# ChanghyeonKim93/bundle_adjustment_solver

Hardware: AMD Instinct MI355X
Metric: lm_iterations_per_sec (higher is better)
Workload: dtype f64; 1 GPU; C4 stereo 6-DoF: 1000 poses / 500k landmarks / 5M obs; n_opt_poses=995, n_opt_landmarks=500000, n_observations=5000000, parallelism=single GPU, exchange=none

## Files before the change

bundle_adjustment_solver_amd/_lib.py:

```python
import ctypes as C
import os

_HERE = os.path.dirname(os.path.abspath(__file__))
LIB_PATH = os.environ.get("BA_HIP_LIB") or os.path.join(_HERE, "libba_hip.so")


class BaOptions(C.Structure):
    _fields_ = [
        ("threshold_step_size", C.c_float),
        ("threshold_cost_change", C.c_float),
        ("threshold_huber_loss", C.c_float),
        ("threshold_outlier_rejection", C.c_float),
        ("max_num_iterations", C.c_int),
        ("initial_lambda", C.c_float),
        ("decrease_ratio_lambda", C.c_float),
        ("increase_ratio_lambda", C.c_float),
        ("gauss_newton", C.c_int),
    ]


def make_options(max_iter=50, thr_step=1e-5, thr_cost=1e-5, huber=1.0,
                 outlier=2.0, lambda0=100.0, dec=0.33, inc=3.0,
                 gauss_newton=False):
    o = BaOptions()
# ... 99 lines not shown
    "ba_solve_gd": (C.c_int, [_P, C.POINTER(BaOptions), C.POINTER(BaIterInfo),
                              C.c_int, C.POINTER(C.c_int), C.POINTER(C.c_int)]),
    "ba_gd_get_gradient": (C.c_int, [_P, _D, _D]),
    "ba_stage_cost": (C.c_int, [_P, _D]),
    "ba_stage_linearize": (C.c_int, [_P, C.c_double, C.c_double]),
    "ba_stage_schur": (C.c_int, [_P]),
    "ba_stage_solve_reduced": (C.c_int, [_P]),
    "ba_stage_backsub_update": (C.c_int, [_P]),
    "ba_stage_scalars": (C.c_int, [_P, _D, _D, _D, _D]),
    "ba_stage_commit": (C.c_int, [_P, C.c_int]),
    "ba_enable_stage_timing": (C.c_int, [_P, C.c_int]),
    "ba_get_stage_ms": (C.c_int, [_P, _D, C.c_int]),
    "ba_num_opt_poses": (C.c_int, [_P]),
    "ba_num_opt_points": (C.c_int, [_P]),
    "ba_num_pairs": (C.c_int64, [_P]),
    "ba_num_schur_blocks": (C.c_int64, [_P]),
    "ba_num_schur_triples": (C.c_int64, [_P]),
    "ba_get_poses": (C.c_int, [_P, _D]),
    "ba_get_points": (C.c_int, [_P, _D, _U8]),
    "ba_get_A": (C.c_int, [_P, _D, _D]),
    "ba_get_C": (C.c_int, [_P, _D, _D]),
    "ba_get_Cinv": (C.c_int, [_P, _D, _D]),
    "ba_get_pairs": (C.c_int, [_P, _I32, _I32, _D]),
    "ba_get_S": (C.c_int, [_P, _D, _D]),
    "ba_get_xy": (C.c_int, [_P, _D, _D]),
    "ba_kernel_count": (C.c_int, []),
    "ba_kernel_name": (C.c_char_p, [C.c_int]),
    "ba_get_kernel_ms": (C.c_int, [_P, _D, C.POINTER(C.c_int64), C.c_int]),
    "ba_get_dense_info": (C.c_int, [_P, _D]),
    "ba_get_schur_info": (C.c_int, [_P, C.POINTER(C.c_int64)]),
    "ba_get_lin_info": (C.c_int, [_P, C.POINTER(C.c_int64)]),
    "ba_get_mask_info": (C.c_int, [_P, C.POINTER(C.c_int64)]),
    "ba_get_dropped_pivots": (C.c_int, [_P, C.POINTER(C.c_int64), C.c_int]),
    "ba_dense_spd_solve": (C.c_int, [_P, C.c_int, _D, _D, _D, _D]),
    "ba_pose_only_mono6": (C.c_int, [_P, _F, _F, C.c_int, C.c_float, C.c_float,
                                     C.c_float, C.c_float, _F, _U8,
                                     C.POINTER(BaOptions), C.POINTER(BaPoIter),
                                     C.c_int, C.POINTER(C.c_int),
                                     C.POINTER(C.c_int), _F]),
    "ba_pose_only_stereo6": (C.c_int, [_P, _F, _F, _F, C.c_int, _F, _F, _F, _F,
                                       _U8, _U8, C.POINTER(BaOptions),
                                       C.POINTER(BaPoIter), C.c_int,
                                       C.POINTER(C.c_int), C.POINTER(C.c_int),
                                       _F]),
    "ba_pose_only_mono3": (C.c_int, [_P, _F, _F, C.c_int, C.c_float, C.c_float,
                                     C.c_float, C.c_float, _F, _F, _F, _U8,
                                     C.POINTER(BaOptions), C.POINTER(BaPoIter),
                                     C.c_int, C.POINTER(C.c_int),
                                     C.POINTER(C.c_int), _F]),
    "ba_pose_only_stereo3": (C.c_int, [_P, _F, _F, _F, C.c_int, _F, _F, _F, _F,
                                       _F, _F, _U8, _U8, C.POINTER(BaOptions),
                                       C.POINTER(BaPoIter), C.c_int,
                                       C.POINTER(C.c_int), C.POINTER(C.c_int),
                                       _F]),
    "ba_pose_only_mono6_batch": (C.c_int, [_P, C.c_int, _I32, _F, _F, _F, _F, _U8,
                                           C.POINTER(BaOptions), C.POINTER(BaPoIter),
                                           C.c_int, C.POINTER(BaPoResult), _F]),
    "ba_pose_only_stereo6_batch": (C.c_int, [_P, C.c_int, _I32, _F, _F, _F, _F, _F,
                                             _F, _F, _U8, _U8, C.POINTER(BaOptions),
                                             C.POINTER(BaPoIter), C.c_int,
                                             C.POINTER(BaPoResult), _F]),
    "ba_pose_only_mono6_batch_device": (C.c_int, [_P, C.c_int, _P, _P, _P, _P, _P, _P,
                                                  C.POINTER(BaOptions), _P, C.c_int,
                                                  _P, _P, _P]),
    "ba_pose_only_stereo6_batch_device": (C.c_int, [_P, C.c_int, _P, _P, _P, _P, _P, _P,
                                                    _P, _P, _P, C.POINTER(BaOptions),
# ... 69 lines not shown
```

bundle_adjustment_solver_amd/csrc/ba_api.hip:

```cpp
#include <hip/hip_runtime.h>

#include <algorithm>
#include <chrono>
#include <cmath>
#include <cstdio>
#include <cstdlib>
#include <cstring>
#include <string>
#include <vector>

#include "ba_handle.h"

namespace {
thread_local std::string g_err;
}
void ba::set_last_error(const std::string &m) { g_err = m; }
int ba::fail(const std::string &m) {
  g_err = m;
  return -1;
}
using ba::fail;

namespace {

// ... 493 lines not shown
    if (h->dalloc(&d.grp_pat, pl.grp_pat.size() / 2) || h->upload(&d.pose_gpart_ptr, pl.pose_gpart_ptr) ||
        h->upload(&d.pose_gpart, pl.pose_gpart))
      return -1;
    h->kind(2);
    if (h->dalloc(&d.Apart2, (size_t)pl.n_apart2 * 27) || h->dalloc(&d.lin_dump, (size_t)ba::kLinDump)) return -1;
    if (!pl.grp_pat.empty())
      HIP_TRY(hipMemcpy(d.grp_pat, pl.grp_pat.data(), pl.grp_pat.size() * sizeof(int32_t), hipMemcpyHostToDevice));
    if (pl.n_apart2 > 0) HIP_TRY(hipMemset(d.Apart2, 0, (size_t)pl.n_apart2 * 27 * sizeof(double)));
  }

  lap("structure uploads");
  for (int k = 0; k < 2; ++k) {
    h->kind(2);
    if (h->dalloc(&d.Cu[k], (size_t)pl.M * 6) || h->dalloc(&d.b[k], (size_t)pl.M * 3) ||
        h->dalloc(&d.W[k], std::max<size_t>(2, (size_t)pl.P * ba::kWStride)))
      return -1;
    h->kind(0);
    if (h->dalloc(&d.A[k], (size_t)pl.N * 36) || h->dalloc(&d.a[k], (size_t)pl.N * 6)) return -1;
    HIP_TRY(hipMemset(d.W[k], 0, std::max<size_t>(1, (size_t)pl.P * ba::kWStride) * sizeof(double)));
    HIP_TRY(hipMemset(d.A[k], 0, std::max<size_t>(1, (size_t)pl.N * 36) * sizeof(double)));
    HIP_TRY(hipMemset(d.a[k], 0, std::max<size_t>(1, (size_t)pl.N * 6) * sizeof(double)));
  }
  d.n_obs_lm = pl.M > 0 ? pl.lm_obs_ptr[pl.M] : 0;
  h->kind(2);
  if (h->dalloc(&d.Cd, (size_t)pl.M * 6) || h->dalloc(&d.Cinv, (size_t)pl.M * 6) ||
      h->dalloc(&d.lin_cost_part, (size_t)std::max(1, d.n_lin_cost)) ||
      h->dalloc(&d.Apart, (size_t)d.n_achunk * 27) ||
      h->dalloc(&d.spart, (size_t)d.n_tchunk * ba::kSlotStride) ||
      h->dalloc(&d.y, (size_t)pl.M * 3) || h->dalloc(&d.lm_part, (size_t)std::max(1, d.n_lm_part) * 2))
    return -1;
  h->kind(0);
  if (h->dalloc(&d.x, (size_t)pl.N * 6 + 64) || h->dalloc(&d.cost_part, (size_t)ba::kCostGrid) ||
      h->dalloc(&d.pose_part, (size_t)2 + 2 * ba::kPoseGrid) ||
      h->dalloc(&d.scal, (size_t)4) || h->dalloc(&d.ctrl, (size_t)1))
    return -1;
  HIP_TRY(hipMemset(d.lin_cost_part, 0, (size_t)std::max(1, d.n_lin_cost) * sizeof(double)));
  HIP_TRY(hipMemset(d.x, 0, ((size_t)pl.N * 6 + 64) * sizeof(double)));
  HIP_TRY(hipMemset(d.y, 0, std::max<size_t>(1, (size_t)pl.M * 3) * sizeof(double)));
  HIP_TRY(hipMemset(d.cost_part, 0, ba::kCostGrid * sizeof(double)));
  HIP_TRY(hipMemset(d.lm_part, 0, (size_t)std::max(1, d.n_lm_part) * 2 * sizeof(double)));
  HIP_TRY(hipMemset(d.pose_part, 0, (2 + 2 * ba::kPoseGrid) * sizeof(double)));
  HIP_TRY(hipMemset(d.scal, 0, 4 * sizeof(double)));
  d.log_cap = 4096;
  if (h->dalloc(&d.log, (size_t)d.log_cap)) return -1;

  lap("block storage");
  if (h->dense_owner) {
    const ba_handle *o = h->dense_owner;
    if (!o->finalized || o->plan.N != pl.N || o->plan.B != pl.B)
      return fail("ba_finalize: the dense owner belongs to a different problem");
    h->sched = o->sched;
    h->ddev = o->ddev;
    h->pose_col_h = o->pose_col_h;
    d.nb = o->d.nb; d.npad = o->d.npad; d.ld = o->d.ld;
    d.L = o->d.L; d.Ldiag = o->d.Ldiag; d.pose_col = o->d.pose_col; d.col_x = o->d.col_x;
    d.zt_I = o->d.zt_I; d.zt_J = o->d.zt_J; d.n_zt = o->d.n_zt;
    d.x = o->d.x;
    h->xbuf_n[0] = pl.B * 36 + 6 * (int64_t)pl.N;
    h->xbuf_n[1] = 4;
    h->xbuf_n[2] = 3 * (int64_t)pl.n_pt_global;
    if (h->dalloc(&d.Spk, (size_t)h->xbuf_n[0])) return -1;
    HIP_TRY(hipMemset(d.Spk, 0, (size_t)h->xbuf_n[0] * sizeof(double)));
  } else {
    const char *nat = getenv("BA_DENSE_NATURAL");
    const char *full = getenv("BA_DENSE_FULL");
    const char *force = getenv("BA_DENSE_NB");
    ba::DenseSchedule cand[2];
    double cost[2];
// ... 805 lines not shown
  for (const auto &g : pl.lin_desc) obs += (int64_t)g.nl * g.no;
  out4[0] = (int64_t)pl.lin_desc.size();
  out4[1] = obs;
  out4[2] = (int64_t)pl.bchunk_lm.size() - 1 - (pl.lin_groups ? pl.n_bchunk_grp : 0);
  out4[3] = pl.n_pobs;
  return 0;
}

int ba_get_mask_info(ba_handle *h, int64_t out4[4]) {
  if (!h || !h->finalized || !out4) return fail("ba_get_mask_info: bad argument");
  const ba::Plan &pl = h->plan;
  int64_t lm = 0;
  for (const auto &g : pl.grp_range) lm += g.masked ? g.nl : 0;
  out4[0] = (int64_t)pl.lin_desc.size() - pl.n_lin_plain;
  out4[1] = lm;
  out4[2] = pl.n_obs - (pl.n_obs_global > 0 && h->world == 1 ? pl.n_obs_global : pl.n_obs);
  {
    int64_t pad = 0;
    for (int64_t s2 = 0; s2 < pl.n_obs; ++s2) pad += !(pl.obs_uv[2 * s2] == pl.obs_uv[2 * s2]);
    out4[2] = pad;
  }
  out4[3] = pl.n_pair_pad;
  return 0;
}

int ba_get_dropped_pivots(ba_handle *h, int64_t *count, int reset) {
  if (!h || !h->finalized || !count) return fail("ba_get_dropped_pivots: bad argument");
  if (use_device(h)) return -1;
  int v = 0;
  HIP_TRY(hipMemcpyAsync(&v, h->ddev.bad_pivots, sizeof(int), hipMemcpyDeviceToHost, h->stream));
  if (reset) HIP_TRY(hipMemsetAsync(h->ddev.bad_pivots, 0, sizeof(int), h->stream));
  HIP_TRY(hipStreamSynchronize(h->stream));
  *count = v % ba::kFlowTimeout;
  return 0;
}

int ba_dense_spd_solve(ba_handle *h, int n, const double *A, const double *b,
                       double *x, double *ms) {
  if (!h || n <= 0 || !A || !b || !x) return fail("ba_dense_spd_solve: bad argument");
  if (use_device(h)) return -1;
  const int nb = 64;
  const int ncb = (n + nb - 1) / nb;
  const int npad = ncb * nb;
  const int ld = npad + nb;
  std::vector<uint8_t> adj((size_t)ncb * ncb, 0);
  for (int I = 0; I < ncb; ++I)
    for (int J = 0; J < I; ++J) {
      bool any = false;
      for (int r = I * nb; r < std::min(n, (I + 1) * nb) && !any; ++r)
        for (int c = J * nb; c < (J + 1) * nb && !any; ++c) any = A[(size_t)r * n + c] != 0.0;
      adj[(size_t)I * ncb + J] = adj[(size_t)J * ncb + I] = any;
    }
  ba::DenseSchedule sc;
  const char *nat = getenv("BA_DENSE_NATURAL");
  ba::build_dense_schedule(ncb, adj, nat && atoi(nat) != 0, nb, sc);
  std::vector<int> colmap(npad), col_x(npad, -1);
  for (int c = 0; c < npad; ++c) colmap[c] = sc.pos_of_tile[c / nb] * nb + c % nb;
  std::vector<double> L((size_t)npad * ld, 0.0);
  for (int c = 0; c < npad; ++c) {
    if (c < n) {
      col_x[colmap[c]] = c;
      for (int r = c; r < n; ++r) {
        int rr = colmap[r], cc = colmap[c];
        if (rr < cc) std::swap(rr, cc);
        L[(size_t)cc * ld + rr] = A[(size_t)r * n + c];
      }
// ... 532 lines not shown
```

bundle_adjustment_solver_amd/csrc/ba_device.h:

```cpp
#ifndef BA_DEVICE_H_
#define BA_DEVICE_H_

#include <hip/hip_runtime.h>
#include <stdint.h>
#include <stdlib.h>

#include <vector>

namespace ba {

struct DevCtrl {
  double lambda;
  double prev_cost;
  double huber;
  double thr_step;
  double thr_cost;
  double dec_ratio;
  double inc_ratio;
  unsigned long long t_last;
  int cur;
  int done;
  int iter;
  int converged;
  int max_iter;
// ... 57 lines not shown
    int32_t pat0;
    int32_t apart0, cost_idx;
    int32_t pad_;
  };
  LinDesc *lin_desc;
  int n_lin_desc;
  int n_lin_plain;
  GrpDesc *grp32, *grp64, *grp128;
  int n_grp32, n_grp64, n_grp128;
  int2 *grp_pat;
  double *Apart2;
  double *lin_dump;
  int32_t *pose_gpart_ptr, *pose_gpart;
  int lin_chunk0;
  int n_lin_cost;
  int n_bs_grp;
  int n_lm_part;
  SupDesc *sup_desc;
  uint32_t *sup_lane;
  ChunkDesc *chunk_desc;
  uint16_t *chunk_sp;
  uint32_t *ltri;
  int64_t *blk_contrib_ptr;
  int32_t *contrib_slot;
  int32_t *blk_desc;
  double *spart2;
  double *Cu[2];
  double *b[2];
  double *W[2];
  double *A[2];
  double *a[2];
  double *Cinv;
  double *Cd;
  double *Apart;
  double *spart;
  double *x;
  double *y;
  double *cost_part;
  double *lin_cost_part;
  int64_t n_obs_lm;
  double *lm_part;
  double *pose_part;
  double *scal;
  DevCtrl *ctrl;
  DevIterRec *log;
  int log_cap;
  double *Spk;
  double *L;
  int npad, ld;
  double *Ldiag;
  int nb;
  int *pose_col;
  int *col_x;
  int32_t *bchunk_lm;
  struct LmChunk {
    int64_t pb, ob;
    int32_t l0, nl, np, no;
  };
  LmChunk *lm_chunk;
  int n_bchunk;
  int *zt_I, *zt_J;
  int n_zt;
};

constexpr int kLinDump = 64 * 4 * 4;
constexpr int kFlowTimeout = 1 << 20;
// ... 175 lines not shown
```

bundle_adjustment_solver_amd/csrc/ba_kernels.hip:

```cpp
#include "ba_device.h"
#include "ba_plan.h"

namespace ba {

thread_local KernelTimer *g_ktimer = nullptr;

void KernelTimer::begin(int id, hipStream_t s) {
  const size_t k = ids.size();
  while (pool.size() < 2 * (k + 1)) {
    hipEvent_t e;
    if (hipEventCreate(&e) != hipSuccess) return;
    pool.push_back(e);
  }
  ids.push_back(id);
  (void)hipEventRecord(pool[2 * k], s);
}
void KernelTimer::end(hipStream_t s) {
  if (ids.empty()) return;
  (void)hipEventRecord(pool[2 * (ids.size() - 1) + 1], s);
}
void KernelTimer::collect() {
  for (size_t k = 0; k < ids.size(); ++k) {
    float t = 0.f;
    if (hipEventElapsedTime(&t, pool[2 * k], pool[2 * k + 1]) == hipSuccess) {
// ... 245 lines not shown
  }
  o[0] = b00; o[1] = b01; o[2] = b02; o[3] = b11; o[4] = b12; o[5] = b22;
}

__device__ __forceinline__ double rcp_newton(double d) {
  double r = __builtin_amdgcn_rcp(d);
  r = fma(fma(-d, r, 1.0), r, r);
  r = fma(fma(-d, r, 1.0), r, r);
  return r;
}
__device__ __forceinline__ void spd3_inverse(const double c[6], double o[6]) {
  const double a00 = c[0], a01 = c[1], a02 = c[2], a11 = c[3], a12 = c[4], a22 = c[5];
  const double thr = 1e-6 * fmax(a00, fmax(a11, a22));
  const double i0 = rcp_newton(a00);
  const double l10 = a01 * i0, l20 = a02 * i0;
  const double d1 = fma(-l10, a01, a11);
  const double t21 = fma(-l20, a01, a12);
  const double i1 = rcp_newton(d1);
  const double l21 = t21 * i1;
  const double d2 = fma(-l21, t21, fma(-l20, a02, a22));
  const double i2 = rcp_newton(d2);
  if (!(a00 > thr && d1 > thr && d2 > thr) || !(thr > 0.0)) {
    ldlt3_inverse(c, o);
    return;
  }
  const double m20 = fma(l10, l21, -l20);
  const double w2 = m20 * i2, v2 = l21 * i2;
  o[5] = i2;
  o[4] = -v2;
  o[2] = w2;
  o[3] = fma(l21, v2, i1);
  o[1] = fma(-l10, i1, -(l21 * w2));
  o[0] = fma(m20, w2, fma(l10 * l10, i1, i0));
}

template <bool SLIM>
struct ObsRec;
template <>
struct ObsRec<true> {
  int2 v;
  __device__ __forceinline__ int cam() const { return v.x & 0xffff; }
  __device__ __forceinline__ int pose() const { return (int)((unsigned)v.x >> 16); }
  __device__ __forceinline__ int pt() const { return v.y; }
  __device__ __forceinline__ void load(const DevProblem &d, int64_t s) { v = d.obs_cp[s]; }
  __device__ __forceinline__ void clear() { v = make_int2(0, 0); }
};
template <>
struct ObsRec<false> {
  int4 v;
  __device__ __forceinline__ int cam() const { return v.x; }
  __device__ __forceinline__ int pose() const { return v.y; }
  __device__ __forceinline__ int pt() const { return v.z; }
  __device__ __forceinline__ void load(const DevProblem &d, int64_t s) { v = d.obs_idx[s]; }
  __device__ __forceinline__ void clear() { v = make_int4(0, 0, 0, 0); }
};

#define COST_STEP(TC, XC, TN, XN)                                               \
  {                                                                             \
             \
    const double *Tp_ = poses + (size_t)idn.pose() * 12;                        \
    const double *Xp_ = pts + (size_t)idn.pt() * 3;                             \
    _Pragma("unroll") for (int k_ = 0; k_ < 12; ++k_) TN[k_] = Tp_[k_];         \
    _Pragma("unroll") for (int k_ = 0; k_ < 3; ++k_) XN[k_] = Xp_[k_];          \
    const int ncam_ = idn.cam();                                                \
    const double2 nuv_ = uvn;                                                   \
     \
// ... 870 lines not shown
    }
    if (k < 18) acc[k] = a2; else racc[k - 18] = a2;
  }
#ifdef BA_SCHUR_DBG
  if (dbg_on)
    for (int k = 0; k < 160; ++k) g_schur_dbg[dbg_slot][k] = k < dbg_n ? dbg_s[k] : 0;
#endif
  if (owner && sub2 == 0) {
    double *o = d.spart2 + (size_t)(sd.s0 + slot) * kSlotStride;
#pragma unroll
    for (int k = 0; k < 18; ++k) o[h * 18 + k] = acc[k];
#pragma unroll
    for (int k = 0; k < 3; ++k) o[36 + h * 3 + k] = racc[k];
  }
}

#ifndef BA_GRP_KRW
#define BA_GRP_KRW 36
#endif
#ifdef BA_GRP_DBG
__device__ long long g_grp_dbg[256];
#define GRP_STAMP() { if (gdbg_on && gdbg_n < 256) gdbg_s[gdbg_n++] = clock64(); }
#else
#define GRP_STAMP()
#endif
template <int NT>
__global__ __launch_bounds__(kBlock, (NT == 2 && BA_GRP_KRW <= 24) ? 3 : 2) void k_schur_grp(DevProblem d, const DevProblem::GrpDesc *grps) {
  constexpr int TW = 16 * NT;
#ifndef BA_GRP_KRW
#define BA_GRP_KRW 36
#endif
  constexpr int KRW = NT == 2 ? BA_GRP_KRW : 20;
  constexpr int NTILE = NT * (NT + 1) / 2;
  constexpr int RS = 2 * TW + (NT == 2 ? 6 : 0);
  constexpr int IMG = (KRW / 2) * RS;
  __shared__ __attribute__((aligned(16))) double VA[4][IMG];
  __shared__ __attribute__((aligned(16))) double WB[4][IMG];
  static_assert(IMG >= 256, "the final reduction uses VA as 4 x 256 doubles");
#ifdef BA_GRP_DBG
  __shared__ long long gdbg_s[256];
  const bool gdbg_on = blockIdx.x == 600 && threadIdx.x == 0;
  int gdbg_n = 0;
#endif
  const int tid = threadIdx.x, lane = tid & 63, wv = tid >> 6;
  const int lr = lane & 15, lk = lane >> 4;
  const DevProblem::GrpDesc gd = grps[blockIdx.x];
  const int done = d.ctrl->done;
  const int lb = d.ctrl->lcur;
  BA_KEEP_S(gd.l0);
  BA_KEEP_S(done);
  if (done) return;
  const double *__restrict__ Wg = d.W[lb];
  const double *__restrict__ bg = d.b[lb];
  const double *__restrict__ Cug = d.Cu[lb];
  const double lp1 = 1.0 + d.ctrl->lambda;
  const int dd = gd.d;
  const int nlw = min(64 / dd, KRW / 3);
  const int il = lane / dd, jj = lane - il * dd;
  const int nch = (gd.nl + nlw - 1) / nlw;
  double *va = VA[wv], *wb = WB[wv];
  for (int e = lane; e < IMG; e += 64) {
    va[e] = 0.0;
    wb[e] = 0.0;
  }
  double2 rw[2][6], rc[2][3];
  double rb[2][3];
#define GRP_PREFETCH(B, ch_)                                                        \
  {                                                                                 \
    const int c0_ = (ch_) * nlw;                                                    \
    const bool on_ = il < min(nlw, gd.nl - c0_);                                    \
    const double2 *wp_ = (const double2 *)(Wg + (size_t)(gd.p0 + (int64_t)c0_ * dd + (on_ ? lane : 0)) * kWStride); \
    const int lm_ = gd.l0 + c0_ + (on_ ? il : 0);                                   \
    const double2 *cp_ = (const double2 *)(Cug + (size_t)lm_ * 6);                  \
    _Pragma("unroll") for (int k_ = 0; k_ < 6; ++k_) rw[B][k_] = wp_[k_];           \
    _Pragma("unroll") for (int k_ = 0; k_ < 3; ++k_) rc[B][k_] = cp_[k_];           \
    _Pragma("unroll") for (int k_ = 0; k_ < 3; ++k_) rb[B][k_] = bg[(size_t)lm_ * 3 + k_]; \
  }
  v4f64 acc[NTILE];
#pragma unroll
  for (int t = 0; t < NTILE; ++t) acc[t] = (v4f64){0.0, 0.0, 0.0, 0.0};
  if (wv < nch) GRP_PREFETCH(0, wv)
  if (wv + 4 < nch) GRP_PREFETCH(1, wv + 4)
#define GRP_IDX(k_, col_) (((k_) >> 1) * RS + (col_) * 2 + ((k_) & 1))
#define GRP_STAGE(B)                                                                \
  if (ch < nch) {                                                                   \
    GRP_STAMP()                                                                     \
    const int nlc = min(nlw, gd.nl - ch * nlw);                                     \
    if (il < nlc) {                                                                 \
       \
      _Pragma("clang fp contract(fast)")                                            \
      const double k9[9] = {rw[B][0].x, rw[B][0].y, rw[B][1].x, rw[B][1].y, rw[B][2].x, \
                            rw[B][2].y, rw[B][3].x, rw[B][3].y, rw[B][4].x};        \
      const double x0 = rw[B][4].y, x1 = rw[B][5].x, x2 = rw[B][5].y;               \
          \
      const double cd_[6] = {rc[B][0].x * lp1, rc[B][0].y, rc[B][1].x, rc[B][1].y * lp1, rc[B][2].x, rc[B][2].y * lp1}; \
      double c6[6];                                                                 \
      spd3_inverse(cd_, c6);                                                        \
      double w[18];                                                                 \
      _Pragma("unroll") for (int e = 0; e < 9; ++e) w[e] = k9[e];                   \
      _Pragma("unroll") for (int c = 0; c < 3; ++c) {                               \
        w[9 + c] = x1 * k9[6 + c] - x2 * k9[3 + c];                                 \
        w[12 + c] = x2 * k9[c] - x0 * k9[6 + c];                                    \
        w[15 + c] = x0 * k9[3 + c] - x1 * k9[c];                                    \
      }                                                                             \
      const int kb = 3 * il, cb = 6 * jj;                                           \
      const int i0 = GRP_IDX(kb, cb), i1 = GRP_IDX(kb + 1, cb), i2 = GRP_IDX(kb + 2, cb); \
      _Pragma("unroll") for (int r = 0; r < 6; ++r) {                               \
        const double w0 = w[r * 3], w1 = w[r * 3 + 1], w2 = w[r * 3 + 2];           \
        va[i0 + 2 * r] = w0 * c6[0] + w1 * c6[1] + w2 * c6[2];                      \
        va[i1 + 2 * r] = w0 * c6[1] + w1 * c6[3] + w2 * c6[4];                      \
        va[i2 + 2 * r] = w0 * c6[2] + w1 * c6[4] + w2 * c6[5];                      \
        wb[i0 + 2 * r] = w0;                                                        \
        wb[i1 + 2 * r] = w1;                                                        \
        wb[i2 + 2 * r] = w2;                                                        \
      }                                                                             \
      if (jj == 0) {                           \
        wb[GRP_IDX(kb, 6 * dd)] = rb[B][0];                                         \
        wb[GRP_IDX(kb + 1, 6 * dd)] = rb[B][1];                                     \
        wb[GRP_IDX(kb + 2, 6 * dd)] = rb[B][2];                                     \
      }                                                                             \
    }                                                                               \
    const int nks = (3 * nlc + 3) >> 2;                                             \
    if (nlc < nlw) {  \
      for (int e = lane; e < (4 * nks - 3 * nlc) * TW; e += 64) {                   \
        const int k_ = 3 * nlc + e / TW, c_ = e - (e / TW) * TW;                    \
        va[GRP_IDX(k_, c_)] = 0.0;                                                  \
        wb[GRP_IDX(k_, c_)] = 0.0;                                                  \
      }                                                                             \
    }                                                                               \
    GRP_STAMP()                                                                     \
    if (ch + 8 < nch) GRP_PREFETCH(B, ch + 8)                                       \
    GRP_STAMP()                                                                     \
    __builtin_amdgcn_fence(__ATOMIC_RELEASE, "wavefront");                          \
    __builtin_amdgcn_wave_barrier();                                                \
    __builtin_amdgcn_fence(__ATOMIC_ACQUIRE, "wavefront");                          \
    {                                                                               \
       \
      const double *ap = va + (lk >> 1) * RS + lr * 2 + (lk & 1);                   \
      const double *bp = wb + (lk >> 1) * RS + lr * 2 + (lk & 1);                   \
      double a[NT], b[NT], an[NT], bn[NT];                                          \
      _Pragma("unroll") for (int t = 0; t < NT; ++t) {                              \
        a[t] = ap[32 * t];                                                          \
        b[t] = bp[32 * t];                                                          \
      }                                                                             \
      for (int ks = 0; ks < nks; ++ks) {                                            \
        const int kn = ks + 1 < nks ? ks + 1 : ks;  \
        _Pragma("unroll") for (int t = 0; t < NT; ++t) {                            \
          an[t] = ap[kn * 2 * RS + 32 * t];                                         \
          bn[t] = bp[kn * 2 * RS + 32 * t];                                         \
        }                                                                           \
        int tile = 0;                                                               \
        _Pragma("unroll") for (int ti = 0; ti < NT; ++ti)                           \
        _Pragma("unroll") for (int tj = ti; tj < NT; ++tj) {                        \
          acc[tile] = __builtin_amdgcn_mfma_f64_16x16x4f64(a[ti], b[tj], acc[tile], 0, 0, 0); \
          ++tile;                                                                   \
        }                                                                           \
        _Pragma("unroll") for (int t = 0; t < NT; ++t) {                            \
          a[t] = an[t];                                                             \
          b[t] = bn[t];                                                             \
        }                                                                           \
      }                                                                             \
    }                                                                               \
    __builtin_amdgcn_fence(__ATOMIC_RELEASE, "wavefront");                          \
    __builtin_amdgcn_wave_barrier();                                                \
    __builtin_amdgcn_fence(__ATOMIC_ACQUIRE, "wavefront");                          \
    GRP_STAMP()                                                                     \
    ch += 4;                                                                        \
  }
  for (int ch = wv; ch < nch;) {
    GRP_STAGE(0)
    GRP_STAGE(1)
  }
#undef GRP_STAGE
#undef GRP_IDX
#undef GRP_PREFETCH
  GRP_STAMP()
#ifdef BA_GRP_DBG
  if (gdbg_on) for (int q = 0; q < 256; ++q) g_grp_dbg[q] = q < gdbg_n ? gdbg_s[q] : 0;
#endif
  __syncthreads();
  double *R = &VA[0][0];
  int tile = 0;
#pragma unroll
  for (int ti = 0; ti < NT; ++ti)
#pragma unroll
    for (int tj = ti; tj < NT; ++tj) {
#pragma unroll
      for (int g = 0; g < 4; ++g) R[wv * 256 + g * 64 + lane] = acc[tile][g];
      __syncthreads();
      {
        const double v = ((R[tid] + R[256 + tid]) + R[512 + tid]) + R[768 + tid];
        const int g = tid >> 6, ln = tid & 63;
        const int row = 16 * ti + (ln >> 4) + 4 * g;
        const int col = 16 * tj + (ln & 15);
        const int pj = row / 6, r = row - 6 * pj;
        if (pj < dd) {
          const int sj = gd.s0 + pj * dd - (pj * (pj - 1)) / 2;
          if (col == 6 * dd) {
            d.spart2[(size_t)sj * kSlotStride + 36 + r] = v;
          } else if (col < 6 * dd) {
            const int pk = col / 6, c = col - 6 * pk;
            if (pk >= pj) d.spart2[(size_t)(sj + (pk - pj)) * kSlotStride + r * 6 + c] = v;
          }
        }
      }
      __syncthreads();
      ++tile;
    }
}

#define GW_LDS_BARRIER() asm volatile("s_waitcnt lgkmcnt(0)\n\ts_barrier" ::: "memory")
__global__ __launch_bounds__(kBlock, 2) void k_schur_grp_wide(DevProblem d, const DevProblem::GrpDesc *grps) {
  constexpr int TW = 128;
  constexpr int LPW = 2;
// ... 1441 lines not shown
```

bundle_adjustment_solver_amd/solver.py:

```python
import ctypes as C
import enum
import sys
import time

import numpy as np

from . import _lib
from ._lib import BaIterInfo, BaOptions, BaPoIter, BaPoResult, check

SCALER = 0.01
INVERSE_SCALER = 1.0 / SCALER


class SolverType(enum.IntEnum):
    UNDEFINED = -1
    GRADIENT_DESCENT = 0
    GAUSS_NEWTON = 1
    LEVENBERG_MARQUARDT = 2


class IterationStatus(enum.IntEnum):
    UNDEFINED = -1
    UPDATE = 0
    UPDATE_TRUST_MORE = 1
# ... 426 lines not shown
        return {self.lib.ba_kernel_name(k).decode(): (float(ms[k]), int(calls[k]))
                for k in range(n)}

    def get_dense_info(self):
        out = np.zeros(4)
        check(self.lib.ba_get_dense_info(self.h, _dp(out)),
              "ba_get_dense_info")
        return dict(fill=out[0], flops=out[1], levels=int(out[2]),
                    npad=int(out[3]))

    def get_schur_info(self):
        v = (C.c_int64 * 8)()
        check(self.lib.ba_get_schur_info(self.h, v), "ba_get_schur_info")
        return dict(groups32=int(v[0]), groups64=int(v[1]), grouped_landmarks=int(v[2]),
                    super_runs=int(v[3]), grouped_pairs=int(v[4]), grouped_triples=int(v[5]),
                    group_mfma=int(v[6]), list_triples=int(v[7]))

    def get_lin_info(self):
        v = (C.c_int64 * 4)()
        check(self.lib.ba_get_lin_info(self.h, v), "ba_get_lin_info")
        return dict(group_pieces=int(v[0]), group_observations=int(v[1]), chunks=int(v[2]),
                    pose_major_observations=int(v[3]))

    def get_mask_info(self):
        v = (C.c_int64 * 4)()
        check(self.lib.ba_get_mask_info(self.h, v), "ba_get_mask_info")
        return dict(masked_pieces=int(v[0]), masked_landmarks=int(v[1]),
                    padded_observation_slots=int(v[2]), padded_pairs=int(v[3]))

    def get_dropped_pivots(self, reset=False):
        v = C.c_int64(0)
        check(self.lib.ba_get_dropped_pivots(self.h, C.byref(v), int(reset)),
              "ba_get_dropped_pivots")
        return int(v.value)

    def dense_spd_solve(self, A, b):
        A = np.ascontiguousarray(A, np.float64)
        b = np.ascontiguousarray(b, np.float64)
        n = A.shape[0]
        x = np.zeros(n)
        ms = C.c_double(0)
        check(self.lib.ba_dense_spd_solve(self.h, n, _dp(A), _dp(b), _dp(x),
                                          C.byref(ms)), "ba_dense_spd_solve")
        return x, ms.value

    def pose_only_mono6(self, X3, uv2, fx, fy, cx, cy, T12, mask, opt,
                        cap=None, want_debug=False):
        X = np.ascontiguousarray(X3, np.float32).reshape(-1, 3)
        uv = np.ascontiguousarray(uv2, np.float32).reshape(-1, 2)
        n = X.shape[0]
        T = np.ascontiguousarray(T12, np.float32).reshape(12).copy()
        m = np.ascontiguousarray(mask, np.uint8).copy()
        cap = cap or max(1, opt.max_num_iterations)
        rows = (BaPoIter * cap)()
        n_it = C.c_int(0)
        conv = C.c_int(0)
        dbg = np.zeros((cap, 12), np.float32) if want_debug else None
        rc = check(self.lib.ba_pose_only_mono6(
            self.h, _fp(X), _fp(uv), n, fx, fy, cx, cy, _fp(T), _up(m),
            C.byref(opt), rows, cap, C.byref(n_it), C.byref(conv),
            _fp(dbg) if want_debug else None), "ba_pose_only_mono6")
        nrows = n_it.value - 1 if conv.value else n_it.value
        nrows = max(0, min(nrows, cap))
        return dict(T12=T, mask=m.astype(bool), n_iter=n_it.value,
                    converged=bool(conv.value), success=(rc == 0),
                    rows=[(rows[i].cost, rows[i].cost_change,
# ... 1191 lines not shown
```

include/ba_hip.h:

```cpp
#ifndef BA_HIP_H_
#define BA_HIP_H_

#include <stdint.h>

#ifdef __cplusplus
extern "C" {
#endif

typedef struct ba_handle ba_handle;

typedef struct {
  float threshold_step_size;
  float threshold_cost_change;
  float threshold_huber_loss;
  float threshold_outlier_rejection;
  int max_num_iterations;
  float initial_lambda;
  float decrease_ratio_lambda;
  float increase_ratio_lambda;
  int gauss_newton;
} ba_options;

typedef struct {
  double cost;
// ... 79 lines not shown
                     double *pose_step_sum, double *point_step_sum);
int ba_stage_commit(ba_handle *h, int accept);

int ba_enable_stage_timing(ba_handle *h, int on);
int ba_get_stage_ms(ba_handle *h, double out8[8], int reset);

int ba_num_opt_poses(ba_handle *h);
int ba_num_opt_points(ba_handle *h);
int64_t ba_num_pairs(ba_handle *h);
int64_t ba_num_schur_blocks(ba_handle *h);
int64_t ba_num_schur_triples(ba_handle *h);
int ba_get_poses(ba_handle *h, double *T_jw12 );
int ba_get_points(ba_handle *h, double *X3 , uint8_t *owned_mask);
int ba_get_A(ba_handle *h, double *A36, double *a6);
int ba_get_C(ba_handle *h, double *C9, double *b3);
int ba_get_Cinv(ba_handle *h, double *Cinv9, double *Cinvb3);
int ba_get_pairs(ba_handle *h, int32_t *pair_i, int32_t *pair_j, double *W18);
int ba_get_S(ba_handle *h, double *S, double *rhs);
int ba_get_xy(ba_handle *h, double *x6, double *y3);

int ba_kernel_count(void);
const char *ba_kernel_name(int id);
int ba_get_kernel_ms(ba_handle *h, double *ms_out, int64_t *calls_out, int reset);

int ba_get_dense_info(ba_handle *h, double out4[4]);

int ba_get_schur_info(ba_handle *h, int64_t out8[8]);

int ba_get_lin_info(ba_handle *h, int64_t out4[4]);

int ba_get_mask_info(ba_handle *h, int64_t out4[4]);

int ba_get_dropped_pivots(ba_handle *h, int64_t *count, int reset);

typedef struct ba_stream ba_stream;
int ba_stream_create(ba_stream **out, int device_id, int n_chunks, int64_t arena_bytes);
void ba_stream_destroy(ba_stream *s);
int ba_stream_set_cameras(ba_stream *s, int n_cam, const double *intr4, const double *T_cj12);
int ba_stream_set_poses(ba_stream *s, int n_pose, const double *T_jw12, const uint8_t *fixed);
int ba_stream_set_points(ba_stream *s, int n_pt, const double *X3, const uint8_t *fixed);
int ba_stream_set_observations(ba_stream *s, int64_t n_obs, const int32_t *cam, const int32_t *pose,
                               const int32_t *point, const double *uv2);
int ba_stream_finalize(ba_stream *s);
int ba_stream_solve(ba_stream *s, const ba_options *opt, ba_iter_info *out, int cap,
                    int *n_iter, int *converged);
int ba_stream_lm_begin(ba_stream *s, const ba_options *opt);
int ba_stream_lm_iterate(ba_stream *s, int n);
int ba_stream_lm_sync(ba_stream *s, ba_iter_info *out, int cap, int *n_iter, int *converged);
int ba_stream_get_poses(ba_stream *s, double *T_jw12);
int ba_stream_get_points(ba_stream *s, double *X3);
int ba_stream_info(ba_stream *s, int64_t out6[6]);

int ba_dense_spd_solve(ba_handle *h, int n, const double *A, const double *b,
                       double *x, double *ms);

typedef struct {
  float cost, cost_change, abs_step;
} ba_po_iter;
int ba_pose_only_mono6(ba_handle *h, const float *X3, const float *uv2, int n,
                       float fx, float fy, float cx, float cy, float *T12,
                       uint8_t *mask, const ba_options *opt, ba_po_iter *iters,
                       int cap, int *n_iter, int *converged,
                       float *debug_T12);

int ba_pose_only_stereo6(ba_handle *h, const float *X3, const float *uvl2,
                         const float *uvr2, int n, const float *intr_l4,
// ... 91 lines not shown
```

Baseline: 2223 it/s.

## Use symmetric Cholesky-factor product for Schur pose-pair tiles with fallback

Rewrites the grouped Schur-complement MFMA kernel so each landmark's damped 3x3 block is factored as L^-T scaled by inverse square roots, letting the pose-pair update be formed as a symmetric product of one shared-memory image instead of two (V and W). A batched per-wave pass computes these factors for several chunks ahead. Chunks whose pivots look ill-conditioned fall back to the old explicit-inverse path, counted through a new device counter and API. This halves shared-memory image traffic and operand loads per MFMA step, at the cost of extra rsqrt work, a second shared buffer and a more complex control path.

```diff
diff --git a/bundle_adjustment_solver_amd/_lib.py b/bundle_adjustment_solver_amd/_lib.py
--- a/bundle_adjustment_solver_amd/_lib.py
+++ b/bundle_adjustment_solver_amd/_lib.py
@@ -155,6 +155,7 @@
     "ba_get_lin_info": (C.c_int, [_P, C.POINTER(C.c_int64)]),
     "ba_get_mask_info": (C.c_int, [_P, C.POINTER(C.c_int64)]),
     "ba_get_dropped_pivots": (C.c_int, [_P, C.POINTER(C.c_int64), C.c_int]),
+    "ba_get_grp_fallback_chunks": (C.c_int, [_P, C.POINTER(C.c_int64), C.c_int]),
     "ba_dense_spd_solve": (C.c_int, [_P, C.c_int, _D, _D, _D, _D]),
     "ba_pose_only_mono6": (C.c_int, [_P, _F, _F, C.c_int, C.c_float, C.c_float,
                                      C.c_float, C.c_float, _F, _U8,
diff --git a/bundle_adjustment_solver_amd/csrc/ba_api.hip b/bundle_adjustment_solver_amd/csrc/ba_api.hip
--- a/bundle_adjustment_solver_amd/csrc/ba_api.hip
+++ b/bundle_adjustment_solver_amd/csrc/ba_api.hip
@@ -549,8 +549,9 @@
   h->kind(0);
   if (h->dalloc(&d.x, (size_t)pl.N * 6 + 64) || h->dalloc(&d.cost_part, (size_t)ba::kCostGrid) ||
       h->dalloc(&d.pose_part, (size_t)2 + 2 * ba::kPoseGrid) ||
-      h->dalloc(&d.scal, (size_t)4) || h->dalloc(&d.ctrl, (size_t)1))
+      h->dalloc(&d.scal, (size_t)4) || h->dalloc(&d.ctrl, (size_t)1) || h->dalloc(&d.grp_fb, (size_t)1))
     return -1;
+  HIP_TRY(hipMemset(d.grp_fb, 0, sizeof(int)));
   HIP_TRY(hipMemset(d.lin_cost_part, 0, (size_t)std::max(1, d.n_lin_cost) * sizeof(double)));
   HIP_TRY(hipMemset(d.x, 0, ((size_t)pl.N * 6 + 64) * sizeof(double)));
   HIP_TRY(hipMemset(d.y, 0, std::max<size_t>(1, (size_t)pl.M * 3) * sizeof(double)));
@@ -1422,6 +1423,17 @@
   if (reset) HIP_TRY(hipMemsetAsync(h->ddev.bad_pivots, 0, sizeof(int), h->stream));
   HIP_TRY(hipStreamSynchronize(h->stream));
   *count = v % ba::kFlowTimeout;
+  return 0;
+}
+
+int ba_get_grp_fallback_chunks(ba_handle *h, int64_t *count, int reset) {
+  if (!h || !h->finalized || !count) return fail("ba_get_grp_fallback_chunks: bad argument");
+  if (use_device(h)) return -1;
+  int v = 0;
+  HIP_TRY(hipMemcpyAsync(&v, h->d.grp_fb, sizeof(int), hipMemcpyDeviceToHost, h->stream));
+  if (reset) HIP_TRY(hipMemsetAsync(h->d.grp_fb, 0, sizeof(int), h->stream));
+  HIP_TRY(hipStreamSynchronize(h->stream));
+  *count = v;
   return 0;
 }
 
diff --git a/bundle_adjustment_solver_amd/csrc/ba_device.h b/bundle_adjustment_solver_amd/csrc/ba_device.h
--- a/bundle_adjustment_solver_amd/csrc/ba_device.h
+++ b/bundle_adjustment_solver_amd/csrc/ba_device.h
@@ -113,6 +113,7 @@
   double *a[2];
   double *Cinv;
   double *Cd;
+  int *grp_fb = nullptr;
   double *Apart;
   double *spart;
   double *x;
diff --git a/bundle_adjustment_solver_amd/csrc/ba_kernels.hip b/bundle_adjustment_solver_amd/csrc/ba_kernels.hip
--- a/bundle_adjustment_solver_amd/csrc/ba_kernels.hip
+++ b/bundle_adjustment_solver_amd/csrc/ba_kernels.hip
@@ -301,6 +301,13 @@
   o[3] = fma(l21, v2, i1);
   o[1] = fma(-l10, i1, -(l21 * w2));
   o[0] = fma(m20, w2, fma(l10 * l10, i1, i0));
+}
+__device__ __forceinline__ double rsq_newton(double x) {
+  double r = __builtin_amdgcn_rsq(x);
+  const double h = 0.5 * x;
+  r = fma(fma(-h * r, r, 0.5), r, r);
+  r = fma(fma(-h * r, r, 0.5), r, r);
+  return r;
 }
 
 template <bool SLIM>
@@ -1237,11 +1244,15 @@
 #endif
   constexpr int KRW = NT == 2 ? BA_GRP_KRW : 20;
   constexpr int NTILE = NT * (NT + 1) / 2;
-  constexpr int RS = 2 * TW + (NT == 2 ? 6 : 0);
+  constexpr int RS = 2 * TW + 6;
   constexpr int IMG = (KRW / 2) * RS;
-  __shared__ __attribute__((aligned(16))) double VA[4][IMG];
-  __shared__ __attribute__((aligned(16))) double WB[4][IMG];
-  static_assert(IMG >= 256, "the final reduction uses VA as 4 x 256 doubles");
+  constexpr int FRS = 10;
+  constexpr int HP = KRW / 4;
+  constexpr int FL = ((KRW / 2) & ~3) / 3;
+  static_assert(KRW % 4 == 0 && FL >= 1, "fallback halves hold whole k steps");
+  __shared__ __attribute__((aligned(16))) double IM[4][IMG];
+  __shared__ __attribute__((aligned(16))) double FR[4][64 * FRS];
+  static_assert(IMG >= 256 && IMG % 2 == 0, "the final reduction uses IM as 4 x 256 doubles");
 #ifdef BA_GRP_DBG
   __shared__ long long gdbg_s[256];
   const bool gdbg_on = blockIdx.x == 600 && threadIdx.x == 0;
@@ -1263,113 +1274,211 @@
   const int nlw = min(64 / dd, KRW / 3);
   const int il = lane / dd, jj = lane - il * dd;
   const int nch = (gd.nl + nlw - 1) / nlw;
-  double *va = VA[wv], *wb = WB[wv];
-  for (int e = lane; e < IMG; e += 64) {
-    va[e] = 0.0;
-    wb[e] = 0.0;
-  }
-  double2 rw[2][6], rc[2][3];
-  double rb[2][3];
+  const int cpb = 64 / nlw;
+  const int fq = lane / nlw, fi = lane - fq * nlw;
+  double *img = IM[wv], *fr = FR[wv];
+  for (int e = lane; e < IMG; e += 64) img[e] = 0.0;
+  double2 rw[2][6];
 #define GRP_PREFETCH(B, ch_)                                                        \
   {                                                                                 \
     const int c0_ = (ch_) * nlw;                                                    \
     const bool on_ = il < min(nlw, gd.nl - c0_);                                    \
     const double2 *wp_ = (const double2 *)(Wg + (size_t)(gd.p0 + (int64_t)c0_ * dd + (on_ ? lane : 0)) * kWStride); \
-    const int lm_ = gd.l0 + c0_ + (on_ ? il : 0);                                   \
+    _Pragma("unroll") for (int k_ = 0; k_ < 6; ++k_) rw[B][k_] = wp_[k_];           \
+  }
+  double2 fc[3];
+  double fb[3];
+#define GRP_FLOAD(ch0_)                                                             \
+  {                                                                                 \
+    const int li_ = ((ch0_) + 4 * fq) * nlw + fi;                                   \
+    const int lm_ = gd.l0 + ((fq < cpb && li_ < gd.nl) ? li_ : 0);                  \
     const double2 *cp_ = (const double2 *)(Cug + (size_t)lm_ * 6);                  \
-    _Pragma("unroll") for (int k_ = 0; k_ < 6; ++k_) rw[B][k_] = wp_[k_];           \
-    _Pragma("unroll") for (int k_ = 0; k_ < 3; ++k_) rc[B][k_] = cp_[k_];           \
-    _Pragma("unroll") for (int k_ = 0; k_ < 3; ++k_) rb[B][k_] = bg[(size_t)lm_ * 3 + k_]; \
+    _Pragma("unroll") for (int k_ = 0; k_ < 3; ++k_) fc[k_] = cp_[k_];              \
+    _Pragma("unroll") for (int k_ = 0; k_ < 3; ++k_) fb[k_] = bg[(size_t)lm_ * 3 + k_]; \
+  }
+  unsigned long long fbad = 0;
+#define GRP_FPASS(ch0_)                                                             \
+  {                                                                                 \
+    const int li_ = ((ch0_) + 4 * fq) * nlw + fi;                                   \
+    const bool on_ = fq < cpb && li_ < gd.nl;                                       \
+    const double a00 = fc[0].x * lp1, a01 = fc[0].y, a02 = fc[1].x;                 \
+    const double a11 = fc[1].y * lp1, a12 = fc[2].x, a22 = fc[2].y * lp1;           \
+    const double thr = 1e-6 * fmax(a00, fmax(a11, a22));                            \
+    const double i0 = rcp_newton(a00);                                              \
+    const double l10 = a01 * i0, l20 = a02 * i0;                                    \
+    const double d1 = fma(-l10, a01, a11);                                          \
+    const double t21 = fma(-l20, a01, a12);                                         \
+    const double i1 = rcp_newton(d1);                                               \
+    const double l21 = t21 * i1;                                                    \
+    const double d2 = fma(-l21, t21, fma(-l20, a02, a22));                          \
+    const bool ok_ = (a00 > thr && d1 > thr && d2 > thr) && thr > 0.0;              \
+    fbad = __ballot(on_ && !ok_);                                                   \
+    const double s0 = rsq_newton(a00), s1 = rsq_newton(d1), s2 = rsq_newton(d2);    \
+    const double m20 = fma(l10, l21, -l20);  \
+    double2 *o_ = (double2 *)(fr + lane * FRS);                                     \
+    o_[0] = make_double2(s0, -l10 * s1);                               \
+    o_[1] = make_double2(m20 * s2, s1);                                \
+    o_[2] = make_double2(-l21 * s2, s2);                               \
+    o_[3] = make_double2(s0 * fb[0], s1 * fma(-l10, fb[0], fb[1]));                 \
+    o_[4] = make_double2(s2 * fma(m20, fb[0], fma(-l21, fb[1], fb[2])), 0.0);       \
+    if ((ch0_) + 4 * cpb < nch) GRP_FLOAD((ch0_) + 4 * cpb)                         \
   }
   v4f64 acc[NTILE];
 #pragma unroll
   for (int t = 0; t < NTILE; ++t) acc[t] = (v4f64){0.0, 0.0, 0.0, 0.0};
   if (wv < nch) GRP_PREFETCH(0, wv)
   if (wv + 4 < nch) GRP_PREFETCH(1, wv + 4)
+  int fpos = cpb;
+  int nfb = 0;
+  if (wv < nch) GRP_FLOAD(wv)
 #define GRP_IDX(k_, col_) (((k_) >> 1) * RS + (col_) * 2 + ((k_) & 1))
+#define GRP_WAVE_SYNC()                                                             \
+  __builtin_amdgcn_fence(__ATOMIC_RELEASE, "wavefront");                            \
+  __builtin_amdgcn_wave_barrier();                                                  \
+  __builtin_amdgcn_fence(__ATOMIC_ACQUIRE, "wavefront");
+  const int opo = (lk >> 1) * RS + lr * 2 + (lk & 1);
+#define GRP_MFMA_SYM(im_, nks_)                                                     \
+  {                                                                                 \
+    const double *ap = (im_) + opo;                                                 \
+    double a[NT], an[NT];                                                           \
+    _Pragma("unroll") for (int t = 0; t < NT; ++t) a[t] = ap[32 * t];               \
+    for (int ks = 0; ks < (nks_); ++ks) {                                           \
+      const int kn = ks + 1 < (nks_) ? ks + 1 : ks;  \
+      _Pragma("unroll") for (int t = 0; t < NT; ++t) an[t] = ap[kn * 2 * RS + 32 * t]; \
+      int tile = 0;                                                                 \
+      _Pragma("unroll") for (int ti = 0; ti < NT; ++ti)                             \
+      _Pragma("unroll") for (int tj = ti; tj < NT; ++tj) {                          \
+        acc[tile] = __builtin_amdgcn_mfma_f64_16x16x4f64(a[ti], a[tj], acc[tile], 0, 0, 0); \
+        ++tile;                                                                     \
+      }                                                                             \
+      _Pragma("unroll") for (int t = 0; t < NT; ++t) a[t] = an[t];                  \
+    }                                                                               \
+  }
+#define GRP_MFMA_VW(va_, wb_, nks_)                                                 \
+  for (int ks = 0; ks < (nks_); ++ks) {                                             \
+    double a[NT], b[NT];                                                            \
+    _Pragma("unroll") for (int t = 0; t < NT; ++t) {                                \
+      a[t] = (va_)[opo + ks * 2 * RS + 32 * t];                                     \
+      b[t] = (wb_)[opo + ks * 2 * RS + 32 * t];                                     \
+    }                                                                               \
+    int tile = 0;                                                                   \
+    _Pragma("unroll") for (int ti = 0; ti < NT; ++ti)                               \
+    _Pragma("unroll") for (int tj = ti; tj < NT; ++tj) {                            \
+      acc[tile] = __builtin_amdgcn_mfma_f64_16x16x4f64(a[ti], b[tj], acc[tile], 0, 0, 0); \
+      ++tile;                                                                       \
+    }                                                                               \
+  }
+#define GRP_FALLBACK(B, nlc_)                                                       \
+  {                                                                                 \
+    for (int e = lane; e < IMG; e += 64) img[e] = 0.0;                              \
+    double *vh = img, *wh = img + HP * RS;                                          \
+    for (int s0 = 0; s0 < (nlc_); s0 += FL) {                                       \
+      const int ns = min(FL, (nlc_) - s0);                                          \
+      if (il >= s0 && il < s0 + ns) {  \
+        _Pragma("clang fp contract(fast)")                                          \
+        const int lm_ = gd.l0 + ch * nlw + il;                                      \
+        const double2 *cp_ = (const double2 *)(Cug + (size_t)lm_ * 6);              \
+        const double2 c01 = cp_[0], c23 = cp_[1], c45 = cp_[2];                     \
+        const double cd_[6] = {c01.x * lp1, c01.y, c23.x, c23.y * lp1, c45.x, c45.y * lp1}; \
+        double c6[6], w[18];                                                        \
+        spd3_inverse(cd_, c6);                                                      \
+        const double k9[9] = {rw[B][0].x, rw[B][0].y, rw[B][1].x, rw[B][1].y, rw[B][2].x, \
+                              rw[B][2].y, rw[B][3].x, rw[B][3].y, rw[B][4].x};      \
+        const double x0 = rw[B][4].y, x1 = rw[B][5].x, x2 = rw[B][5].y;             \
+        _Pragma("unroll") for (int e = 0; e < 9; ++e) w[e] = k9[e];                 \
+        _Pragma("unroll") for (int c = 0; c < 3; ++c) {                             \
+          w[9 + c] = x1 * k9[6 + c] - x2 * k9[3 + c];                               \
+          w[12 + c] = x2 * k9[c] - x0 * k9[6 + c];                                  \
+          w[15 + c] = x0 * k9[3 + c] - x1 * k9[c];                                  \
+        }                                                                           \
+        const int kb = 3 * (il - s0), cb = 6 * jj;                                  \
+        const int i0 = GRP_IDX(kb, cb), i1 = GRP_IDX(kb + 1, cb), i2 = GRP_IDX(kb + 2, cb); \
+        _Pragma("unroll") for (int r = 0; r < 6; ++r) {                             \
+          const double w0 = w[r * 3], w1 = w[r * 3 + 1], w2 = w[r * 3 + 2];         \
+          vh[i0 + 2 * r] = w0 * c6[0] + w1 * c6[1] + w2 * c6[2];                    \
+          vh[i1 + 2 * r] = w0 * c6[1] + w1 * c6[3] + w2 * c6[4];                    \
+          vh[i2 + 2 * r] = w0 * c6[2] + w1 * c6[4] + w2 * c6[5];                    \
+          wh[i0 + 2 * r] = w0;                                                      \
+          wh[i1 + 2 * r] = w1;                                                      \
+          wh[i2 + 2 * r] = w2;                                                      \
+        }                                                                           \
+        if (jj == 0) {                         \
+          wh[GRP_IDX(kb, 6 * dd)] = bg[(size_t)lm_ * 3];                            \
+          wh[GRP_IDX(kb + 1, 6 * dd)] = bg[(size_t)lm_ * 3 + 1];                    \
+          wh[GRP_IDX(kb + 2, 6 * dd)] = bg[(size_t)lm_ * 3 + 2];                    \
+        }                                                                           \
+      }                                                                             \
+      GRP_WAVE_SYNC()                                                               \
+      GRP_MFMA_VW(vh, wh, (3 * ns + 3) >> 2)                                        \
+      GRP_WAVE_SYNC()                                                               \
+      for (int e = lane; e < IMG; e += 64) img[e] = 0.0;                            \
+    }                                                                               \
+  }
 #define GRP_STAGE(B)                                                                \
   if (ch < nch) {                                                                   \
     GRP_STAMP()                                                                     \
+    if (fpos == cpb) {  \
+      GRP_FPASS(ch)                                                                 \
+      GRP_WAVE_SYNC()                         \
+      fpos = 0;                                                                     \
+    }                                                                               \
     const int nlc = min(nlw, gd.nl - ch * nlw);                                     \
-    if (il < nlc) {                                                                 \
-       \
-      _Pragma("clang fp contract(fast)")                                            \
-      const double k9[9] = {rw[B][0].x, rw[B][0].y, rw[B][1].x, rw[B][1].y, rw[B][2].x, \
-                            rw[B][2].y, rw[B][3].x, rw[B][3].y, rw[B][4].x};        \
-      const double x0 = rw[B][4].y, x1 = rw[B][5].x, x2 = rw[B][5].y;               \
-          \
-      const double cd_[6] = {rc[B][0].x * lp1, rc[B][0].y, rc[B][1].x, rc[B][1].y * lp1, rc[B][2].x, rc[B][2].y * lp1}; \
-      double c6[6];                                                                 \
-      spd3_inverse(cd_, c6);                                                        \
-      double w[18];                                                                 \
-      _Pragma("unroll") for (int e = 0; e < 9; ++e) w[e] = k9[e];                   \
-      _Pragma("unroll") for (int c = 0; c < 3; ++c) {                               \
-        w[9 + c] = x1 * k9[6 + c] - x2 * k9[3 + c];                                 \
-        w[12 + c] = x2 * k9[c] - x0 * k9[6 + c];                                    \
-        w[15 + c] = x0 * k9[3 + c] - x1 * k9[c];                                    \
+    if (((fbad >> (fpos * nlw)) & ((1ull << nlc) - 1)) == 0) {                      \
+      if (il < nlc) {                                                               \
+                         \
+        const double2 *g_ = (const double2 *)(fr + (fpos * nlw + il) * FRS);        \
+        const double2 ga = g_[0], gb = g_[1], gc = g_[2];                           \
+        const double k9[9] = {rw[B][0].x, rw[B][0].y, rw[B][1].x, rw[B][1].y, rw[B][2].x, \
+                              rw[B][2].y, rw[B][3].x, rw[B][3].y, rw[B][4].x};      \
+        const double x0 = rw[B][4].y, x1 = rw[B][5].x, x2 = rw[B][5].y;             \
+        double y[18];                                   \
+        _Pragma("unroll") for (int r = 0; r < 3; ++r) {                             \
+          const double q0 = k9[3 * r], q1 = k9[3 * r + 1], q2 = k9[3 * r + 2];      \
+          y[3 * r] = q0 * ga.x;                                                     \
+          y[3 * r + 1] = fma(q0, ga.y, q1 * gb.y);                                  \
+          y[3 * r + 2] = fma(q0, gb.x, fma(q1, gc.x, q2 * gc.y));                   \
+        }                                                                           \
+        _Pragma("unroll") for (int m = 0; m < 3; ++m) {                             \
+          y[9 + m] = fma(x1, y[6 + m], -(x2 * y[3 + m]));                           \
+          y[12 + m] = fma(x2, y[m], -(x0 * y[6 + m]));                              \
+          y[15 + m] = fma(x0, y[3 + m], -(x1 * y[m]));                              \
+        }                                                                           \
+        const int kb = 3 * il, cb = 6 * jj;                                         \
+        const int i0 = GRP_IDX(kb, cb), i1 = GRP_IDX(kb + 1, cb), i2 = GRP_IDX(kb + 2, cb); \
+        _Pragma("unroll") for (int r = 0; r < 6; ++r) {                             \
+          img[i0 + 2 * r] = y[3 * r];                                               \
+          img[i1 + 2 * r] = y[3 * r + 1];                                           \
+          img[i2 + 2 * r] = y[3 * r + 2];                                           \
+        }                                                                           \
+        if (jj == 0) {                                                              \
+          const double2 za = g_[3], zb = g_[4];                                     \
+          img[GRP_IDX(kb, 6 * dd)] = za.x;                                          \
+          img[GRP_IDX(kb + 1, 6 * dd)] = za.y;                                      \
+          img[GRP_IDX(kb + 2, 6 * dd)] = zb.x;                                      \
+        }                                                                           \
       }                                                                             \
-      const int kb = 3 * il, cb = 6 * jj;                                           \
-      const int i0 = GRP_IDX(kb, cb), i1 = GRP_IDX(kb + 1, cb), i2 = GRP_IDX(kb + 2, cb); \
-      _Pragma("unroll") for (int r = 0; r < 6; ++r) {                               \
-        const double w0 = w[r * 3], w1 = w[r * 3 + 1], w2 = w[r * 3 + 2];           \
-        va[i0 + 2 * r] = w0 * c6[0] + w1 * c6[1] + w2 * c6[2];                      \
-        va[i1 + 2 * r] = w0 * c6[1] + w1 * c6[3] + w2 * c6[4];                      \
-        va[i2 + 2 * r] = w0 * c6[2] + w1 * c6[4] + w2 * c6[5];                      \
-        wb[i0 + 2 * r] = w0;                                                        \
-        wb[i1 + 2 * r] = w1;                                                        \
-        wb[i2 + 2 * r] = w2;                                                        \
+      const int nks = (3 * nlc + 3) >> 2;                                           \
+      if (nlc < nlw) {  \
+        for (int e = lane; e < (4 * nks - 3 * nlc) * TW; e += 64) {                 \
+          const int k_ = 3 * nlc + e / TW, c_ = e - (e / TW) * TW;                  \
+          img[GRP_IDX(k_, c_)] = 0.0;                                               \
+        }                                                                           \
       }                                                                             \
-      if (jj == 0) {                           \
-        wb[GRP_IDX(kb, 6 * dd)] = rb[B][0];                                         \
-        wb[GRP_IDX(kb + 1, 6 * dd)] = rb[B][1];                                     \
-        wb[GRP_IDX(kb + 2, 6 * dd)] = rb[B][2];                                     \
-      }                                                                             \
-    }                                                                               \
-    const int nks = (3 * nlc + 3) >> 2;                                             \
-    if (nlc < nlw) {  \
-      for (int e = lane; e < (4 * nks - 3 * nlc) * TW; e += 64) {                   \
-        const int k_ = 3 * nlc + e / TW, c_ = e - (e / TW) * TW;                    \
-        va[GRP_IDX(k_, c_)] = 0.0;                                                  \
-        wb[GRP_IDX(k_, c_)] = 0.0;                                                  \
-      }                                                                             \
+      GRP_STAMP()                                                                   \
+      if (ch + 8 < nch) GRP_PREFETCH(B, ch + 8)                                     \
+      GRP_STAMP()                                                                   \
+      GRP_WAVE_SYNC()                                                               \
+      GRP_MFMA_SYM(img, nks)                                                        \
+      GRP_WAVE_SYNC()                                                               \
+    } else {     \
+      GRP_FALLBACK(B, nlc)                                                          \
+      GRP_STAMP()                                                                   \
+      if (ch + 8 < nch) GRP_PREFETCH(B, ch + 8)                                     \
+      GRP_STAMP()                                                                   \
+      ++nfb;                                                                        \
     }                                                                               \
     GRP_STAMP()                                                                     \
-    if (ch + 8 < nch) GRP_PREFETCH(B, ch + 8)                                       \
-    GRP_STAMP()                                                                     \
-    __builtin_amdgcn_fence(__ATOMIC_RELEASE, "wavefront");                          \
-    __builtin_amdgcn_wave_barrier();                                                \
-    __builtin_amdgcn_fence(__ATOMIC_ACQUIRE, "wavefront");                          \
-    {                                                                               \
-       \
-      const double *ap = va + (lk >> 1) * RS + lr * 2 + (lk & 1);                   \
-      const double *bp = wb + (lk >> 1) * RS + lr * 2 + (lk & 1);                   \
-      double a[NT], b[NT], an[NT], bn[NT];                                          \
-      _Pragma("unroll") for (int t = 0; t < NT; ++t) {                              \
-        a[t] = ap[32 * t];                                                          \
-        b[t] = bp[32 * t];                                                          \
-      }                                                                             \
-      for (int ks = 0; ks < nks; ++ks) {                                            \
-        const int kn = ks + 1 < nks ? ks + 1 : ks;  \
-        _Pragma("unroll") for (int t = 0; t < NT; ++t) {                            \
-          an[t] = ap[kn * 2 * RS + 32 * t];                                         \
-          bn[t] = bp[kn * 2 * RS + 32 * t];                                         \
-        }                                                                           \
-        int tile = 0;                                                               \
-        _Pragma("unroll") for (int ti = 0; ti < NT; ++ti)                           \
-        _Pragma("unroll") for (int tj = ti; tj < NT; ++tj) {                        \
-          acc[tile] = __builtin_amdgcn_mfma_f64_16x16x4f64(a[ti], b[tj], acc[tile], 0, 0, 0); \
-          ++tile;                                                                   \
-        }                                                                           \
-        _Pragma("unroll") for (int t = 0; t < NT; ++t) {                            \
-          a[t] = an[t];                                                             \
-          b[t] = bn[t];                                                             \
-        }                                                                           \
-      }                                                                             \
-    }                                                                               \
-    __builtin_amdgcn_fence(__ATOMIC_RELEASE, "wavefront");                          \
-    __builtin_amdgcn_wave_barrier();                                                \
-    __builtin_amdgcn_fence(__ATOMIC_ACQUIRE, "wavefront");                          \
-    GRP_STAMP()                                                                     \
+    ++fpos;                                                                         \
     ch += 4;                                                                        \
   }
   for (int ch = wv; ch < nch;) {
@@ -1377,14 +1486,21 @@
     GRP_STAGE(1)
   }
 #undef GRP_STAGE
+#undef GRP_FALLBACK
+#undef GRP_MFMA_VW
+#undef GRP_MFMA_SYM
+#undef GRP_WAVE_SYNC
+#undef GRP_FPASS
+#undef GRP_FLOAD
 #undef GRP_IDX
 #undef GRP_PREFETCH
   GRP_STAMP()
 #ifdef BA_GRP_DBG
   if (gdbg_on) for (int q = 0; q < 256; ++q) g_grp_dbg[q] = q < gdbg_n ? gdbg_s[q] : 0;
 #endif
+  if (nfb > 0 && lane == 0 && d.grp_fb) atomicAdd(d.grp_fb, nfb);
   __syncthreads();
-  double *R = &VA[0][0];
+  double *R = &IM[0][0];
   int tile = 0;
 #pragma unroll
   for (int ti = 0; ti < NT; ++ti)
diff --git a/bundle_adjustment_solver_amd/solver.py b/bundle_adjustment_solver_amd/solver.py
--- a/bundle_adjustment_solver_amd/solver.py
+++ b/bundle_adjustment_solver_amd/solver.py
@@ -482,6 +482,12 @@
         v = C.c_int64(0)
         check(self.lib.ba_get_dropped_pivots(self.h, C.byref(v), int(reset)),
               "ba_get_dropped_pivots")
+        return int(v.value)
+
+    def get_grp_fallback_chunks(self, reset=False):
+        v = C.c_int64(0)
+        check(self.lib.ba_get_grp_fallback_chunks(self.h, C.byref(v), int(reset)),
+              "ba_get_grp_fallback_chunks")
         return int(v.value)
 
     def dense_spd_solve(self, A, b):
diff --git a/include/ba_hip.h b/include/ba_hip.h
--- a/include/ba_hip.h
+++ b/include/ba_hip.h
@@ -135,6 +135,8 @@
 int ba_get_mask_info(ba_handle *h, int64_t out4[4]);
 
 int ba_get_dropped_pivots(ba_handle *h, int64_t *count, int reset);
+
+int ba_get_grp_fallback_chunks(ba_handle *h, int64_t *count, int reset);
 
 typedef struct ba_stream ba_stream;
 int ba_stream_create(ba_stream **out, int device_id, int n_chunks, int64_t arena_bytes);
```

After: 2358 it/s, median of 6. +6.1%, better.
